# pkuyzy/ESC-GNN

Measured on AMD Instinct MI355X. Metric: graphs/sec + edges-aggregated/sec, NestedGIN_eff h=3 bs=128 @1/2/4/8 GPU, higher is better.
Workload: dtype f32; 1 GPU; count_cycle-shaped random regular graphs (n in 10/15/20/30), target=triangles, NestedGIN_eff h=3 layers=4 hidden=256, bs=128 per GPU (configs[1]); global_batch=128, parallelism=dp1 graph-sharded, rccl_ranks=1, ranks=1

## Files before the change

### esc-gnn_amd/csrc/linear_mfma.hip

```cpp
#include "common.h"
#include <cstdlib>
#include "linear_plan.h"
#include "gemm_tile.h"
#include "gemm_dma.h"
#include "linear_small.h"
#include "linear_narrow.h"

namespace esc {

using plan::Flags;
using plan::Op;
using plan::Plan;

static plan::PlanKnobs g_plan;
void set_linear_knob(int knob, int value) {
  if (knob == 11) g_plan.use_dma = value;
  else g_plan.knob[knob] = value;
}
static const plan::PlanKnobs& knobs() {
  static const bool env_read = [] {
    if (getenv("ESC_BIG_MIN_WGS")) g_plan.big_min_wgs = atoll(getenv("ESC_BIG_MIN_WGS"));
    if (getenv("ESC_TILE160")) g_plan.tile160 = atoi(getenv("ESC_TILE160"));
    if (getenv("ESC_TILE160_MIN_WGS")) g_plan.tile160_min_wgs = atoll(getenv("ESC_TILE160_MIN_WGS"));
    return true;
// ... 74 lines not shown
static void dma_fill_dw(dma::GArgs& g, const float* dY, int64_t ld_dy, const float* X, int64_t ld_x, const float* in_scale,
                        const float* in_shift, int64_t M, int64_t N, int64_t K, float* slabs, const Plan& p) {
  g.A = dY; g.lda = (int)ld_dy; g.B = X; g.ldb = (int)ld_x; g.C = slabs; g.ldc = (int)K;
  g.pro_scale = in_scale; g.pro_shift = in_shift; g.db_part = slabs + (size_t)p.splits * N * K;
  g.M = (int)N; g.N = (int)K; g.R = (int)M; g.red_per_split = p.per_split; g.accumulate = 0;
}

enum NarrowForm { NARROW_PLAIN, NARROW_FOLD, NARROW_L1 };
static void launch_narrow_fwd(NarrowForm form, const float* X, int64_t ld_x, const float* W, int64_t ld_w, const float* bias,
                              const float* in_scale, const float* in_shift, int64_t M, int64_t N, int64_t K, float* Y, int64_t ld_y,
                              const BnFoldDev& fold, const NarrowL1& l1, hipStream_t s) {
  const unsigned blocks = (unsigned)(cdiv(M, 16) < 2048 ? cdiv(M, 16) : 2048);
#define ESC_NARROW_FWD(...) \
  esc::launch(ESC_K_LINEAR, linear_narrow_fwd<__VA_ARGS__>, dim3(blocks), dim3(256), 0, s, X, ld_x, W, ld_w, bias, in_scale, in_shift, (int)M, (int)N, (int)K, Y, ld_y, fold, l1)
  if (form == NARROW_L1) ESC_NARROW_FWD(1, true, false, true);
  else if (form == NARROW_FOLD) { if (N == 1) ESC_NARROW_FWD(1, true, true); else ESC_NARROW_FWD(4, true, true); }
  else if (N == 1) { if (in_scale) ESC_NARROW_FWD(1, true); else ESC_NARROW_FWD(1, false); }
  else { if (in_scale) ESC_NARROW_FWD(4, true); else ESC_NARROW_FWD(4, false); }
#undef ESC_NARROW_FWD
}

static hipError_t launch_dma_fwd(const Plan& p, const dma::GArgs& g, hipStream_t s) {
  const bool pro = g.pro_scale != nullptr;
#define ESC_DMA_FWD(PRO, ...) dma::launch_gemm<__VA_ARGS__, false, false, PRO, true, false>(g, 0, s)
#define ESC_DMA_FWD_FROM(PRO, ...) dma::launch_gemm<__VA_ARGS__, false, false, PRO, true, false, true>(g, 0, s)
  const bool big = p.family == plan::F_DMA128;
  if (g.c_init != nullptr) {
    if (big) return pro ? ESC_DMA_FWD_FROM(1, ESC_T128) : ESC_DMA_FWD_FROM(0, ESC_T128);
    return pro ? ESC_DMA_FWD_FROM(1, ESC_T64) : ESC_DMA_FWD_FROM(0, ESC_T64);
  }
  if (g.fold.partials != nullptr) return big ? ESC_DMA_FWD(3, ESC_T128) : ESC_DMA_FWD(3, ESC_T64);
  switch (p.family) {
    case plan::F_DMA64X32:
      return pro ? dma::launch_gemm<ESC_T64X32, false, false, 1, false, false>(g, 0, s)
                 : dma::launch_gemm<ESC_T64X32, false, false, 0, false, false>(g, 0, s);
    case plan::F_DMA160: return pro ? ESC_DMA_FWD(1, ESC_T160) : ESC_DMA_FWD(0, ESC_T160);
    case plan::F_DMA128: return pro ? ESC_DMA_FWD(1, ESC_T128) : ESC_DMA_FWD(0, ESC_T128);
    case plan::F_DMA128X64: return ESC_DMA_FWD(0, ESC_T128X64);
    default: return pro ? ESC_DMA_FWD(1, ESC_T64) : ESC_DMA_FWD(0, ESC_T64);
  }
#undef ESC_DMA_FWD
#undef ESC_DMA_FWD_FROM
}
static dma::GArgs dma_fwd_args(const float* X, int64_t ld_x, const float* W, int64_t ld_w, const float* bias, const float* in_scale,
                               const float* in_shift, int64_t M, int64_t N, int64_t K, float* Y, int64_t ld_y, float* col_stats) {
  dma::GArgs g{};
  g.A = X; g.lda = (int)ld_x; g.B = W; g.ldb = (int)ld_w; g.C = Y; g.ldc = (int)ld_y; g.bias = bias;
  g.pro_scale = in_scale; g.pro_shift = in_shift; g.col_stats = reinterpret_cast<float2*>(col_stats);
  g.M = (int)M; g.N = (int)N; g.R = (int)K; g.red_per_split = (int)K; g.accumulate = 0;
  return g;
}

static int launch_smalln_dx(const float* dY, int64_t ld_dy, const float* W, int64_t ld_w, int64_t M, int64_t N, int64_t K, float* dX,
                            int64_t ld_dx, int accumulate, const BnbDev& bd, int act, const char* what, hipStream_t s) {
  const size_t lds = (size_t)(32 + small::SMALL_MAX) * (N + 4) * sizeof(float);
  static size_t raised[3] = {64 * 1024, 64 * 1024, 64 * 1024};
  hipError_t e = hipSuccess;
  if (act == 0) e = dma::raise_lds(small::smalln_dx<small::SMALL_MAX>, lds, raised[0]);
  if (act != 0) e = dma::raise_lds(small::smalln_dx<small::SMALL_MAX, 1>, lds, raised[1]);
  if (e == hipSuccess && act == 2) e = dma::raise_lds(small::smalln_dx<small::SMALL_MAX, 2>, lds, raised[2]);
  if (dma_check(e, what) != hipSuccess) return ESC_ELAUNCH;
  auto kern = act == 0 ? small::smalln_dx<small::SMALL_MAX> : (act == 2 ? small::smalln_dx<small::SMALL_MAX, 2> : small::smalln_dx<small::SMALL_MAX, 1>);
  esc::launch(ESC_K_LINEAR, kern, dim3((unsigned)cdiv(M, 32)), dim3(256), lds, s, dY, ld_dy, W, ld_w, (int)M, (int)N, (int)K, dX, ld_dx, accumulate, bd);
  return ESC_OK;
}

static void launch_wgrad_small(const float* dY, int64_t ld_dy, const float* X, int64_t ld_x, const float* in_scale, const float* in_shift,
                               int64_t M, int64_t N, int64_t K, float* slabs, const Plan& p, const BnbDev& bd, int act, hipStream_t s) {
  float* db_part = slabs + (size_t)p.splits * N * K;
  const bool small_k = K <= small::SMALL_MAX;
  const dim3 grid((unsigned)p.splits, (unsigned)cdiv(small_k ? N : K, 256));
#define ESC_WGRAD_SMALL(...) \
  esc::launch(ESC_K_LINEAR, small::wgrad_small<small::SMALL_MAX, __VA_ARGS__>, grid, dim3(256), 0, s, dY, ld_dy, X, ld_x, in_scale, in_shift, (int)M, (int)N, (int)K, slabs, db_part, bd)
  if (act == 2)      { if (in_scale) ESC_WGRAD_SMALL(true, true, 2); else ESC_WGRAD_SMALL(true, false, 2); }
  else if (act == 1) { if (in_scale) ESC_WGRAD_SMALL(true, true, 1); else ESC_WGRAD_SMALL(true, false, 1); }
  else if (small_k)  { if (in_scale) ESC_WGRAD_SMALL(true, true); else ESC_WGRAD_SMALL(true, false); }
  else               { if (in_scale) ESC_WGRAD_SMALL(false, true); else ESC_WGRAD_SMALL(false, false); }
#undef ESC_WGRAD_SMALL
}

static int reduce_slabs(const Plan& p, const float* slabs, int64_t N, int64_t K, float* dW, int64_t ld_dw, float* db, esc_reduce_job* defer,
                        void* stream) {
  esc_reduce_job now;
  esc_reduce_job* j = defer ? defer : &now;
  j->slabs = slabs; j->n = N * K; j->splits = p.splits; j->cols = K; j->dw = dW; j->ld_dw = ld_dw;
  j->db_part = slabs + (size_t)p.splits * N * K; j->rows = N; j->db = db;
  return defer ? ESC_OK : esc_slab_reduce_jobs(j, 1, stream);
}

}

using namespace esc;

extern "C" {

int esc_debug_gemm_occupancy(int tile_id) {
  int n = -1;
#define ESC_OCC(I)                                                                                                              \
  {                                                                                                                             \
    constexpr plan::Tile t = plan::R01_TILE[I];                                                                                 \
    auto kern = gemm_tile_kernel<t.bm, t.bn, t.wm, t.wn, t.bk, true, true, false, false>;                                       \
    const size_t lds = 2 * (KContigTile<t.bm, t.bk>::FLOATS + KContigTile<t.bn, t.bk>::FLOATS) * sizeof(float);                 \
    if (lds > 64 * 1024) (void)hipFuncSetAttribute((const void*)kern, hipFuncAttributeMaxDynamicSharedMemorySize, (int)lds);    \
    (void)hipOccupancyMaxActiveBlocksPerMultiprocessor(&n, kern, 256, lds);                                                     \
  }
  switch (tile_id) {
    case 0: ESC_OCC(0) break;
    case 2: ESC_OCC(2) break;
    case 3: ESC_OCC(3) break;
    case 4: ESC_OCC(4) break;
    default: ESC_OCC(1) break;
  }
#undef ESC_OCC
  return n;
}

static int linear_fwd_impl(const float* X, int64_t ld_x, const float* W, int64_t ld_w, const float* bias,
                           const float* in_scale, const float* in_shift, int64_t M, int64_t N, int64_t K,
                           float* Y, int64_t ld_y, float* col_stats, const esc_bn_fuse* bn, void* stream) {
  ESC_REQUIRE(X && W && Y, "esc_linear_fwd: null pointer");
  ESC_REQUIRE(M >= 0 && N > 0 && K > 0 && ld_x >= K && ld_w >= K && ld_y >= N, "esc_linear_fwd: bad sizes M=%ld N=%ld K=%ld", (long)M, (long)N, (long)K);
  ESC_REQUIRE((in_scale == nullptr) == (in_shift == nullptr), "esc_linear_fwd: in_scale/in_shift must come together");
  ESC_REQUIRE(col_stats == nullptr || N > 32, "esc_linear_fwd: col_stats needs N > 32");
  ESC_REQUIRE(M < (1LL << 31) && N < (1LL << 31) && K < (1LL << 31), "esc_linear_fwd: dimension too large");
  ESC_REQUIRE(bn == nullptr || (col_stats && bn->mean && bn->invstd && M > 1), "esc_linear_bn_fwd: needs col_stats, mean, invstd and M > 1");
  ESC_REQUIRE(bn == nullptr || ((bn->scale == nullptr) == (bn->shift == nullptr)), "esc_linear_bn_fwd: scale/shift must come together");
  if (M == 0) return ESC_OK;
  hipStream_t s = (hipStream_t)stream;
  Flags f = pro_flags(in_scale, in_shift);
  f.col_stats = col_stats != nullptr; f.bn = bn != nullptr; f.last_block_finalize = last_block_finalize();
  const Plan p = plan::plan_fwd(knobs(), Op{X, ld_x}, Op{W, ld_w}, M, N, K, f);
// ... 94 lines not shown
int esc_linear_fwd_from(const float* Y0, int64_t ld_y0, const float* X, int64_t ld_x, const float* W, int64_t ld_w, const float* bias,
                        const float* in_scale, const float* in_shift, int64_t M, int64_t N, int64_t K, float* Y, int64_t ld_y,
                        float* col_stats, void* stream) {
  ESC_REQUIRE(Y0 && X && W && Y, "esc_linear_fwd_from: null pointer");
  ESC_REQUIRE(M > 0 && N > 32 && K >= 32 && ld_y0 >= N && ld_x >= K && ld_w >= K && ld_y >= N && M < (1LL << 31), "esc_linear_fwd_from: bad sizes");
  ESC_REQUIRE((in_scale == nullptr) == (in_shift == nullptr), "esc_linear_fwd_from: in_scale/in_shift must come together");
  Flags f = pro_flags(in_scale, in_shift);
  f.c_init = true; f.col_stats = col_stats != nullptr;
  const Plan p = plan::plan_fwd(knobs(), Op{X, ld_x}, Op{W, ld_w}, M, N, K, f);
  ESC_REQUIRE(p.ok, "esc_linear_fwd_from: shape not served by the LDS-DMA tiles (M=%ld N=%ld K=%ld)", (long)M, (long)N, (long)K);
  dma::GArgs g = dma_fwd_args(X, ld_x, W, ld_w, bias, in_scale, in_shift, M, N, K, Y, ld_y, col_stats);
  g.c_init = Y0; g.ld_init = (int)ld_y0;
  return dma_check(launch_dma_fwd(p, g, (hipStream_t)stream), "esc_linear_fwd_from") == hipSuccess ? ESC_OK : ESC_ELAUNCH;
}
int esc_linear_fwd_from_ok(const float* X, int64_t ld_x, const float* W, int64_t ld_w, int64_t M, int64_t N, int64_t K, int has_prologue) {
  Flags f;
  f.pro = has_prologue != 0; f.c_init = true;
  return plan::plan_fwd(knobs(), Op{X, ld_x}, Op{W, ld_w}, M, N, K, f).ok ? 1 : 0;
}

int esc_linear_fwd_l1_ok(const float* X, int64_t ld_x, const float* w, int64_t K, const float* in_scale, const float* in_shift) {
  return (in_scale && in_shift && plan::plan_fwd(knobs(), Op{X, ld_x}, Op{w, K}, 1, 1, K, pro_flags(in_scale, in_shift)).family == plan::F_NARROW) ? 1 : 0;
}
int esc_linear_fwd_l1(const float* X, int64_t ld_x, const float* w, const float* bias, const float* in_scale, const float* in_shift,
                      int64_t M, int64_t K, const float* target, int64_t denom, float grad_scale, float* pred, float* dpred, void* stream) {
  ESC_REQUIRE(X && w && target && pred && dpred, "esc_linear_fwd_l1: null pointer");
  ESC_REQUIRE(M > 0 && K > 0 && ld_x >= K && denom > 0 && M < (1LL << 31), "esc_linear_fwd_l1: bad sizes");
  ESC_REQUIRE(in_scale != nullptr && in_shift != nullptr, "esc_linear_fwd_l1: the head reads pre-BatchNorm rows (in_scale / in_shift)");
  ESC_REQUIRE(esc_linear_fwd_l1_ok(X, ld_x, w, K, in_scale, in_shift), "esc_linear_fwd_l1: shape / alignment not served (K=%ld)", (long)K);
  const NarrowL1 l1{target, (float)((double)grad_scale / (double)denom), dpred};
  launch_narrow_fwd(NARROW_L1, X, ld_x, w, K, bias, in_scale, in_shift, M, 1, K, pred, 1, BnFoldDev{}, l1, (hipStream_t)stream);
  ESC_CHECK_LAUNCH("esc_linear_fwd_l1");
  return ESC_OK;
}

int esc_linear_bwd_input(const float* dY, int64_t ld_dy, const float* W, int64_t ld_w, int64_t M,
                         int64_t N, int64_t K, float* dX, int64_t ld_dx, int accumulate,
                         void* stream) {
  ESC_REQUIRE(dY && W && dX, "esc_linear_bwd_input: null pointer");
  ESC_REQUIRE(M >= 0 && N > 0 && K > 0 && ld_dy >= N && ld_w >= K && ld_dx >= K, "esc_linear_bwd_input: bad sizes");
  ESC_REQUIRE(M < (1LL << 31) && N < (1LL << 31) && K < (1LL << 31), "esc_linear_bwd_input: dimension too large");
  if (M == 0) return ESC_OK;
  hipStream_t s = (hipStream_t)stream;
  const Plan p = plan::plan_dx(knobs(), Op{dY, ld_dy}, Op{W, ld_w}, Op{dX, ld_dx}, M, N, K);
  switch (p.family) {
    case plan::F_NARROW_DX: {
      const unsigned blocks = (unsigned)(cdiv(M, 16) < 4096 ? cdiv(M, 16) : 4096);
      if (p.bn == 4) esc::launch(ESC_K_LINEAR, linear_narrow_dx<4>, dim3(blocks), dim3(256), 0, s, dY, ld_dy, W, ld_w, (int)M, (int)N, (int)K, dX, ld_dx, accumulate);
      else           esc::launch(ESC_K_LINEAR, linear_narrow_dx<16>, dim3(blocks), dim3(256), 0, s, dY, ld_dy, W, ld_w, (int)M, (int)N, (int)K, dX, ld_dx, accumulate);
      ESC_CHECK_LAUNCH("esc_linear_bwd_input.narrow");
      return ESC_OK;
    }
    case plan::F_SMALLN_DX:
      ESC_TRY_(launch_smalln_dx(dY, ld_dy, W, ld_w, M, N, K, dX, ld_dx, accumulate, BnbDev{}, 0, "esc_linear_bwd_input", s));
      ESC_CHECK_LAUNCH("esc_linear_bwd_input.smalln");
      return ESC_OK;
    case plan::F_DMA160_DX: case plan::F_DMA128_DX: case plan::F_DMA64_DX: {
      dma::GArgs d{};
      dma_fill_dx(d, dY, ld_dy, W, ld_w, M, N, K, dX, ld_dx, accumulate);
      const hipError_t e = p.family == plan::F_DMA160_DX   ? dma::launch_gemm<ESC_T160, false, true, 0, false, false>(d, 0, s)
                           : p.family == plan::F_DMA128_DX ? dma::launch_gemm<ESC_T128, false, true, 0, false, false>(d, 0, s)
                                                           : dma::launch_gemm<ESC_T64, false, true, 0, false, false>(d, 0, s);
      return dma_check(e, "esc_linear_bwd_input") == hipSuccess ? ESC_OK : ESC_ELAUNCH;
    }
    default:
      launch_r01<true, false, false, false>(p.tile, r01_dx_args(dY, ld_dy, W, ld_w, M, N, K, dX, ld_dx, accumulate), 1, s);
      ESC_CHECK_LAUNCH("esc_linear_bwd_input");
      return ESC_OK;
  }
}

int64_t esc_linear_bwd_weight_scratch(int64_t M, int64_t N, int64_t K) { return plan::bwd_weight_scratch(M, N, K); }

static int weight_impl(const float* dY, int64_t ld_dy, const float* X, int64_t ld_x, const float* in_scale,
                       const float* in_shift, int64_t M, int64_t N, int64_t K, float* dW, int64_t ld_dw, float* db,
                       float* slabs, esc_reduce_job* defer, void* stream) {
  ESC_REQUIRE(dY && X && dW && slabs, "esc_linear_bwd_weight: null pointer");
  ESC_REQUIRE(M > 0 && N > 0 && K > 0 && ld_dy >= N && ld_x >= K && ld_dw >= K, "esc_linear_bwd_weight: bad sizes");
  ESC_REQUIRE((in_scale == nullptr) == (in_shift == nullptr), "esc_linear_bwd_weight: in_scale/in_shift must come together");
  ESC_REQUIRE(M < (1LL << 31) && N < (1LL << 31) && K < (1LL << 31), "esc_linear_bwd_weight: dimension too large");
  hipStream_t s = (hipStream_t)stream;
  const Plan p = plan::plan_dw(knobs(), Op{dY, ld_dy}, Op{X, ld_x}, slabs, M, N, K);
  switch (p.family) {
    case plan::F_SMALL_DW:
      launch_wgrad_small(dY, ld_dy, X, ld_x, in_scale, in_shift, M, N, K, slabs, p, BnbDev{}, 0, s);
      ESC_CHECK_LAUNCH("esc_linear_bwd_weight.small");
      break;
    case plan::F_DMA128_DW: case plan::F_DMA64_DW: {
      dma::GArgs d{};
      dma_fill_dw(d, dY, ld_dy, X, ld_x, in_scale, in_shift, M, N, K, slabs, p);
      hipError_t e;
      if (p.family == plan::F_DMA128_DW) e = in_scale ? dma::launch_gemm<ESC_T128, true, true, 2, false, true>(d, 0, s)
                                                      : dma::launch_gemm<ESC_T128, true, true, 0, false, true>(d, 0, s);
      else                               e = in_scale ? dma::launch_gemm<ESC_T64, true, true, 2, false, true>(d, 0, s)
                                                      : dma::launch_gemm<ESC_T64, true, true, 0, false, true>(d, 0, s);
      if (dma_check(e, "esc_linear_bwd_weight") != hipSuccess) return ESC_ELAUNCH;
      break;
    }
    default: {
      const GemmArgs g = r01_dw_args(dY, ld_dy, X, ld_x, in_scale, in_shift, M, N, K, slabs, p);
      if (in_scale) launch_r01<false, false, true, true>(p.tile, g, p.splits, s);
      else          launch_r01<false, false, false, true>(p.tile, g, p.splits, s);
      ESC_CHECK_LAUNCH("esc_linear_bwd_weight.tiles");
    }
  }
  return reduce_slabs(p, slabs, N, K, dW, ld_dw, db, defer, stream);
}

int esc_linear_bwd_weight(const float* dY, int64_t ld_dy, const float* X, int64_t ld_x,
                          const float* in_scale, const float* in_shift, int64_t M, int64_t N,
                          int64_t K, float* dW, int64_t ld_dw, float* db, float* slabs,
                          void* stream) {
  return weight_impl(dY, ld_dy, X, ld_x, in_scale, in_shift, M, N, K, dW, ld_dw, db, slabs, nullptr, stream);
}

int esc_slab_reduce_jobs(const esc_reduce_job* jobs, int count, void* stream) {
  ESC_REQUIRE(jobs && count > 0 && count <= ESC_MAX_REDUCE_JOBS, "esc_slab_reduce_jobs: 1..%d jobs", ESC_MAX_REDUCE_JOBS);
  ReduceJobs t{};
  t.count = count;
  int blocks = 0;
  for (int j = 0; j < count; ++j) {
    ESC_REQUIRE(jobs[j].slabs && jobs[j].dw && jobs[j].n > 0 && jobs[j].splits > 0, "esc_slab_reduce_jobs: bad job %d", j);
    t.job[j] = jobs[j];
    t.block_start[j] = blocks;
    const esc_reduce_job& q = jobs[j];
    const bool vec = q.n % 4 == 0 && q.cols % 4 == 0 && q.ld_dw % 4 == 0 && aligned16(q.slabs) && aligned16(q.dw);
    t.vec[j] = vec ? 1 : 0;
    blocks += (int)(cdiv(vec ? q.n / 4 : q.n, 64) + (q.db ? cdiv(q.rows, 64) : 0));
  }
  t.block_start[count] = blocks;
  esc::launch(ESC_K_LINEAR, slab_reduce_multi_kernel, dim3((unsigned)blocks), dim3(256), 0, (hipStream_t)stream, t);
  ESC_CHECK_LAUNCH("esc_slab_reduce_jobs");
  return ESC_OK;
}

static int both_impl(const float* dY, int64_t ld_dy, const float* X, int64_t ld_x, const float* in_scale,
                     const float* in_shift, const float* W, int64_t ld_w, int64_t M, int64_t N, int64_t K,
                     float* dX, int64_t ld_dx, int accumulate, float* dW, int64_t ld_dw, float* db,
// ... 48 lines not shown
  }
  return reduce_slabs(p, slabs, N, K, dW, ld_dw, db, defer, stream);
}

int esc_linear_bwd_both(const float* dY, int64_t ld_dy, const float* X, int64_t ld_x, const float* in_scale,
                        const float* in_shift, const float* W, int64_t ld_w, int64_t M, int64_t N, int64_t K,
                        float* dX, int64_t ld_dx, int accumulate, float* dW, int64_t ld_dw, float* db,
                        float* slabs, void* stream) {
  return both_impl(dY, ld_dy, X, ld_x, in_scale, in_shift, W, ld_w, M, N, K, dX, ld_dx, accumulate, dW, ld_dw, db, slabs,
                   nullptr, stream);
}

int esc_linear_bwd_both_deferred(const float* dY, int64_t ld_dy, const float* X, int64_t ld_x, const float* in_scale,
                                 const float* in_shift, const float* W, int64_t ld_w, int64_t M, int64_t N, int64_t K,
                                 float* dX, int64_t ld_dx, int accumulate, float* dW, int64_t ld_dw, float* db,
                                 float* slabs, esc_reduce_job* job, void* stream) {
  ESC_REQUIRE(job, "esc_linear_bwd_both_deferred: null job");
  return both_impl(dY, ld_dy, X, ld_x, in_scale, in_shift, W, ld_w, M, N, K, dX, ld_dx, accumulate, dW, ld_dw, db, slabs,
                   job, stream);
}

static Plan plan_both_bn(const float* dOut, int64_t ld_dout, const esc_bn_bwd_fused* b, const float* X, int64_t ld_x, const float* W,
                         int64_t ld_w, int64_t M, int64_t N, int64_t K, const float* dX, int64_t ld_dx, const float* slabs,
                         const esc_bn_bwd_next* n) {
  plan::BnOps bo{};
  plan::NextOps no{};
  if (b) bo = plan::BnOps{b->x, b->ld_x, b->mean, b->invstd, b->scale, b->shift, b->coef, b->relu};
  if (n) no = plan::NextOps{n->partial, n->x, n->ld_x, n->mean, n->invstd, n->scale, n->shift, n->relu};
  return plan::plan_both_bn(knobs(), Op{dOut, ld_dout}, b ? &bo : nullptr, Op{X, ld_x}, Op{W, ld_w}, Op{dX, ld_dx}, slabs, n ? &no : nullptr,
                            M, N, K);
}

int esc_linear_bwd_both_bn_ok(const float* dOut, int64_t ld_dout, const esc_bn_bwd_fused* bn, const float* X, int64_t ld_x,
                              const float* W, int64_t ld_w, int64_t M, int64_t N, int64_t K, const float* dX, int64_t ld_dx,
                              const float* slabs, const esc_bn_bwd_next* next) {
  return plan_both_bn(dOut, ld_dout, bn, X, ld_x, W, ld_w, M, N, K, dX, ld_dx, slabs, next).ok ? 1 : 0;
}

int64_t esc_linear_bwd_bn_block_rows(int64_t M, int64_t N, int64_t K) { return plan::bwd_bn_block_rows(M, N, K); }

int esc_linear_bwd_both_bn(const float* dOut, int64_t ld_dout, const esc_bn_bwd_fused* bn, const float* X, int64_t ld_x,
                           const float* in_scale, const float* in_shift, const float* W, int64_t ld_w, int64_t M,
                           int64_t N, int64_t K, float* dX, int64_t ld_dx, int accumulate, float* dW, int64_t ld_dw,
                           float* db, float* slabs, esc_reduce_job* defer, const esc_bn_bwd_next* next, void* stream) {
  ESC_REQUIRE(dOut && X && W && dW && slabs, "esc_linear_bwd_both_bn: null pointer");
  ESC_REQUIRE((in_scale == nullptr) == (in_shift == nullptr), "esc_linear_bwd_both_bn: in_scale/in_shift must come together");
  ESC_REQUIRE(ld_dw >= K, "esc_linear_bwd_both_bn: bad sizes");
  const Plan p = plan_both_bn(dOut, ld_dout, bn, X, ld_x, W, ld_w, M, N, K, dX, ld_dx, slabs, next);
  ESC_REQUIRE(p.ok, "esc_linear_bwd_both_bn: shape / alignment not served (M=%ld N=%ld K=%ld) - use esc_bn_bwd + esc_linear_bwd_both", (long)M, (long)N, (long)K);
  hipStream_t s = (hipStream_t)stream;
  const BnbDev bd = bn ? BnbDev{bn->x, (int)bn->ld_x, bn->mean, bn->invstd, bn->scale, bn->shift, reinterpret_cast<const float2*>(bn->coef), bn->relu}
                       : BnbDev{};
  if (p.family == plan::F_SMALL_BN) {
    const int act = bd.relu == 2 ? 2 : 1;
    launch_wgrad_small(dOut, ld_dout, X, ld_x, in_scale, in_shift, M, N, K, slabs, p, bd, act, s);
    ESC_CHECK_LAUNCH("esc_linear_bwd_both_bn.small");
    if (dX != nullptr) {
      ESC_TRY_(launch_smalln_dx(dOut, ld_dout, W, ld_w, M, N, K, dX, ld_dx, accumulate, bd, act, "esc_linear_bwd_both_bn", s));
      ESC_CHECK_LAUNCH("esc_linear_bwd_both_bn.smalln");
    }
    return reduce_slabs(p, slabs, N, K, dW, ld_dw, db, defer, stream);
  }
  dma::DualArgs a{};
  dma_fill_dx(a.dx, dOut, ld_dout, W, ld_w, M, N, K, dX, ld_dx, accumulate);
  dma_fill_dw(a.dw, dOut, ld_dout, X, ld_x, in_scale, in_shift, M, N, K, slabs, p);
  a.dx.bnb = bd; a.dw.bnb = bd;
  if (next)
    a.dx.bst = BnStatDev{reinterpret_cast<float2*>(next->partial), next->x, (int)next->ld_x, next->mean, next->invstd, next->scale, next->shift, next->relu};
  hipError_t e;
#define ESC_T64_2STAGE 64, 64, 32, 2, 2, 2, 2
  if (p.family == plan::F_DMA128_BN) {
    if (next) e = in_scale ? dma::launch_dual<ESC_T128, true, true, true>(a, 0, s) : dma::launch_dual<ESC_T128, false, true, true>(a, 0, s);
    else      e = in_scale ? dma::launch_dual<ESC_T128, true, true, false>(a, 0, s) : dma::launch_dual<ESC_T128, false, true, false>(a, 0, s);
  } else {
    if (bn == nullptr) e = in_scale ? dma::launch_dual<ESC_T64, true, false, true>(a, 0, s) : dma::launch_dual<ESC_T64, false, false, true>(a, 0, s);
    else if (next)     e = in_scale ? dma::launch_dual<ESC_T64_2STAGE, true, true, true>(a, 0, s) : dma::launch_dual<ESC_T64_2STAGE, false, true, true>(a, 0, s);
    else               e = in_scale ? dma::launch_dual<ESC_T64_2STAGE, true, true, false>(a, 0, s) : dma::launch_dual<ESC_T64_2STAGE, false, true, false>(a, 0, s);
  }
#undef ESC_T64_2STAGE
  if (dma_check(e, "esc_linear_bwd_both_bn") != hipSuccess) return ESC_ELAUNCH;
  return reduce_slabs(p, slabs, N, K, dW, ld_dw, db, defer, stream);
}

}
```

### esc-gnn_amd/csrc/linear_small.h

```cpp
#pragma once
#include "common.h"
#include "linear_plan.h"

namespace esc {
namespace small {


template <int KMAX>
__global__ __launch_bounds__(256) void smallk_fwd(const float* __restrict__ X, int64_t ldx, const float* __restrict__ W,
                                                  int64_t ldw, const float* __restrict__ bias, int M, int N, int K,
                                                  float* __restrict__ Y, int64_t ldy, float2* __restrict__ col_stats) {
  ESC_PRIO();
  __shared__ float xs[ROWS_FWD * KMAX];
  const int n = blockIdx.y * 256 + threadIdx.x;
  const int r0 = blockIdx.x * ROWS_FWD;
  const int rows = min(ROWS_FWD, M - r0);
  for (int i = threadIdx.x; i < ROWS_FWD * KMAX; i += 256) {
    const int r = i / KMAX, k = i % KMAX;
    xs[i] = (r < rows && k < K) ? X[(size_t)(r0 + r) * ldx + k] : 0.f;
  }
  float w[KMAX];
#pragma unroll
  for (int k = 0; k < KMAX; ++k) w[k] = (n < N && k < K) ? W[(size_t)n * ldw + k] : 0.f;
  const float b = (bias != nullptr && n < N) ? bias[n] : 0.f;
  __syncthreads();
  if (n >= N) return;
  float y[ROWS_FWD];
  float s1 = 0.f;
#pragma unroll
  for (int r = 0; r < ROWS_FWD; ++r) {
    float a = b;
#pragma unroll
    for (int k = 0; k < KMAX; ++k) a = fmaf(xs[r * KMAX + k], w[k], a);
    y[r] = a;
    if (r < rows) { Y[(size_t)(r0 + r) * ldy + n] = a; s1 += a; }
  }
  if (col_stats != nullptr) {
    const float mean = s1 / (float)rows;
    float m2 = 0.f;
#pragma unroll
    for (int r = 0; r < ROWS_FWD; ++r)
      if (r < rows) { const float d = y[r] - mean; m2 = fmaf(d, d, m2); }
    col_stats[(size_t)blockIdx.x * N + n] = make_float2(mean, m2);
  }
}

template <int SMAX, bool SMALL_K, bool PRO, int BNB = 0>
__global__ __launch_bounds__(256) void wgrad_small(const float* __restrict__ dY, int64_t lddy, const float* __restrict__ X,
                                                   int64_t ldx, const float* __restrict__ sc, const float* __restrict__ sh,
                                                   int M, int N, int K, float* __restrict__ slabs, float* __restrict__ db_part,
                                                   BnbDev bnb) {
  static_assert(BNB == 0 || SMALL_K, "the fused BatchNorm backward transforms the wide dY operand");
  ESC_PRIO();
  __shared__ float us[ROWS_WGRAD * SMAX];
  const int t = blockIdx.y * 256 + threadIdx.x;
  const int split = blockIdx.x;
  const int r0 = split * ROWS_WGRAD;
  const int rows = min(ROWS_WGRAD, M - r0);
  const int S = SMALL_K ? K : N;
  const int Wd = SMALL_K ? N : K;
  const float* U = SMALL_K ? X : dY;
  const int64_t ldu = SMALL_K ? ldx : lddy;
  for (int i = threadIdx.x; i < rows * S; i += 256) {
    float v = U[(size_t)(r0 + i / S) * ldu + (i % S)];
    if constexpr (PRO && SMALL_K) v = fmaxf(fmaf(v, sc[i % S], sh[i % S]), 0.f);
    us[(i / S) * SMAX + (i % S)] = v;
  }
  for (int i = threadIdx.x; i < ROWS_WGRAD * SMAX; i += 256)
    if (i / SMAX >= rows || i % SMAX >= S) us[i] = 0.f;
  __syncthreads();
  float acc[SMAX];
#pragma unroll
  for (int q = 0; q < SMAX; ++q) acc[q] = 0.f;
  float colsum = 0.f;
  if (t < Wd) {
    const float* V = SMALL_K ? dY : X;
    const int64_t ldv = SMALL_K ? lddy : ldx;
    float psc = 1.f, psh = 0.f;
    if constexpr (PRO && !SMALL_K) { psc = sc[t]; psh = sh[t]; }
    float b_mu = 0.f, b_a = 0.f, b_ms = 0.f, b_mh = 1.f, b_k1 = 0.f, b_k2 = 0.f;
    if constexpr (BNB != 0) {
      const float2 kk = bnb.coef[t];
      b_mu = bnb.mean[t]; b_a = bnb.scale[t]; b_k1 = kk.x; b_k2 = bnb.invstd[t] * kk.y;
      if (bnb.relu) { b_ms = b_a; b_mh = bnb.shift[t]; }
    }
#pragma unroll 4
    for (int r = 0; r < rows; ++r) {
      float v = V[(size_t)(r0 + r) * ldv + t];
      if constexpr (BNB == 1) v = bnb_apply(v, bnb.x[(size_t)(r0 + r) * bnb.ldx + t], b_mu, b_a, b_ms, b_mh, b_k1, b_k2);
      if constexpr (BNB == 2) v = bnb_apply_elu(v, bnb.x[(size_t)(r0 + r) * bnb.ldx + t], b_mu, b_a, b_ms, b_mh, b_k1, b_k2);
      if constexpr (PRO && !SMALL_K) v = fmaxf(fmaf(v, psc, psh), 0.f);
      if constexpr (SMALL_K) colsum += v;
#pragma unroll
      for (int q = 0; q < SMAX; ++q) acc[q] = fmaf(us[r * SMAX + q], v, acc[q]);
    }
    float* out = slabs + (size_t)split * N * K;
#pragma unroll
    for (int q = 0; q < SMAX; ++q)
      if (q < S) out[SMALL_K ? (size_t)t * K + q : (size_t)q * K + t] = acc[q];
    if constexpr (SMALL_K) db_part[(size_t)split * N + t] = colsum;
  }
  if constexpr (!SMALL_K) {
    if (blockIdx.y == 0 && (int)threadIdx.x < N) {
      float s = 0.f;
      for (int r = 0; r < rows; ++r) s += us[r * SMAX + threadIdx.x];
      db_part[(size_t)split * N + threadIdx.x] = s;
    }
  }
}

template <int KMAX, int BNB = 0>
__global__ __launch_bounds__(256) void smalln_dx(const float* __restrict__ dY, int64_t lddy, const float* __restrict__ W,
                                                 int64_t ldw, int M, int N, int K, float* __restrict__ dX, int64_t lddx,
                                                 int accumulate, BnbDev bnb) {
  ESC_PRIO();
  extern __shared__ __attribute__((aligned(16))) float sm[];
  const int ldn = N + 4;
  float* ys = sm;
  float* wt = sm + 32 * ldn;
  const int r0 = blockIdx.x * 32;
  const int rows = min(32, M - r0);
  for (int i = threadIdx.x; i < rows * (N / 4); i += 256) {
    const int r = i / (N / 4), c = (i % (N / 4)) * 4;
    float4 v = *reinterpret_cast<const float4*>(dY + (size_t)(r0 + r) * lddy + c);
    if constexpr (BNB != 0) {
      const float4 x = *reinterpret_cast<const float4*>(bnb.x + (size_t)(r0 + r) * bnb.ldx + c);
      const float4 mu = *reinterpret_cast<const float4*>(bnb.mean + c), a = *reinterpret_cast<const float4*>(bnb.scale + c);
      const float4 is = *reinterpret_cast<const float4*>(bnb.invstd + c);
      const float4 k01 = *reinterpret_cast<const float4*>(bnb.coef + c), k23 = *reinterpret_cast<const float4*>(bnb.coef + c + 2);
      float4 ms = make_float4(0.f, 0.f, 0.f, 0.f), mh = make_float4(1.f, 1.f, 1.f, 1.f);
      if (bnb.relu) { ms = a; mh = *reinterpret_cast<const float4*>(bnb.shift + c); }
      if constexpr (BNB == 2) {
        v.x = bnb_apply_elu(v.x, x.x, mu.x, a.x, ms.x, mh.x, k01.x, is.x * k01.y); v.y = bnb_apply_elu(v.y, x.y, mu.y, a.y, ms.y, mh.y, k01.z, is.y * k01.w);
        v.z = bnb_apply_elu(v.z, x.z, mu.z, a.z, ms.z, mh.z, k23.x, is.z * k23.y); v.w = bnb_apply_elu(v.w, x.w, mu.w, a.w, ms.w, mh.w, k23.z, is.w * k23.w);
      } else {
        v.x = bnb_apply(v.x, x.x, mu.x, a.x, ms.x, mh.x, k01.x, is.x * k01.y); v.y = bnb_apply(v.y, x.y, mu.y, a.y, ms.y, mh.y, k01.z, is.y * k01.w);
        v.z = bnb_apply(v.z, x.z, mu.z, a.z, ms.z, mh.z, k23.x, is.z * k23.y); v.w = bnb_apply(v.w, x.w, mu.w, a.w, ms.w, mh.w, k23.z, is.w * k23.w);
      }
    }
    *reinterpret_cast<float4*>(ys + r * ldn + c) = v;
  }
  for (int i = threadIdx.x; i < N * K; i += 256) wt[(i % K) * ldn + (i / K)] = W[(size_t)(i / K) * ldw + (i % K)];
  __syncthreads();
  const int r = threadIdx.x >> 3, ks = threadIdx.x & 7;
  if (r >= rows) return;
#pragma unroll
  for (int kk = 0; kk < KMAX / 8; ++kk) {
    const int k = ks + kk * 8;
    if (k >= K) break;
    float a0 = 0.f, a1 = 0.f, a2 = 0.f, a3 = 0.f;
    for (int c = 0; c < N; c += 4) {
      const float4 y = *reinterpret_cast<const float4*>(ys + r * ldn + c);
      const float4 w = *reinterpret_cast<const float4*>(wt + k * ldn + c);
      a0 = fmaf(y.x, w.x, a0); a1 = fmaf(y.y, w.y, a1); a2 = fmaf(y.z, w.z, a2); a3 = fmaf(y.w, w.w, a3);
    }
    float v = (a0 + a1) + (a2 + a3);
    float* dst = dX + (size_t)(r0 + r) * lddx + k;
    if (accumulate) v += *dst;
    *dst = v;
  }
}

}
}
```

Before: 134,100 graphs/s.

## Fuse BatchNorm-backward weight and input gradients into one small-K kernel

Replaces the separate wgrad_small and smalln_dx launches on the BatchNorm-fused small path with a single bn_both kernel. It applies the BN backward transform to dOut once into LDS, computes the weight-gradient slab and bias partials, then reuses the transformed rows to compute dX against W staged in LDS. This avoids a second launch and re-reading dOut and the BN input x from global memory. Separately, the plain wgrad_small kernel now preloads its row values into registers ahead of the LDS staging. The cost is a larger LDS footprint per block and more register pressure.

```diff
diff --git a/esc-gnn_amd/csrc/linear_mfma.hip b/esc-gnn_amd/csrc/linear_mfma.hip
--- a/esc-gnn_amd/csrc/linear_mfma.hip
+++ b/esc-gnn_amd/csrc/linear_mfma.hip
@@ -150,31 +150,45 @@
 }
 
 static int launch_smalln_dx(const float* dY, int64_t ld_dy, const float* W, int64_t ld_w, int64_t M, int64_t N, int64_t K, float* dX,
-                            int64_t ld_dx, int accumulate, const BnbDev& bd, int act, const char* what, hipStream_t s) {
+                            int64_t ld_dx, int accumulate, const char* what, hipStream_t s) {
   const size_t lds = (size_t)(32 + small::SMALL_MAX) * (N + 4) * sizeof(float);
-  static size_t raised[3] = {64 * 1024, 64 * 1024, 64 * 1024};
-  hipError_t e = hipSuccess;
-  if (act == 0) e = dma::raise_lds(small::smalln_dx<small::SMALL_MAX>, lds, raised[0]);
-  if (act != 0) e = dma::raise_lds(small::smalln_dx<small::SMALL_MAX, 1>, lds, raised[1]);
-  if (e == hipSuccess && act == 2) e = dma::raise_lds(small::smalln_dx<small::SMALL_MAX, 2>, lds, raised[2]);
-  if (dma_check(e, what) != hipSuccess) return ESC_ELAUNCH;
-  auto kern = act == 0 ? small::smalln_dx<small::SMALL_MAX> : (act == 2 ? small::smalln_dx<small::SMALL_MAX, 2> : small::smalln_dx<small::SMALL_MAX, 1>);
-  esc::launch(ESC_K_LINEAR, kern, dim3((unsigned)cdiv(M, 32)), dim3(256), lds, s, dY, ld_dy, W, ld_w, (int)M, (int)N, (int)K, dX, ld_dx, accumulate, bd);
+  static size_t raised = 64 * 1024;
+  if (dma_check(dma::raise_lds(small::smalln_dx<small::SMALL_MAX>, lds, raised), what) != hipSuccess) return ESC_ELAUNCH;
+  esc::launch(ESC_K_LINEAR, small::smalln_dx<small::SMALL_MAX>, dim3((unsigned)cdiv(M, 32)), dim3(256), lds, s, dY, ld_dy, W, ld_w, (int)M, (int)N,
+              (int)K, dX, ld_dx, accumulate);
   return ESC_OK;
 }
 
 static void launch_wgrad_small(const float* dY, int64_t ld_dy, const float* X, int64_t ld_x, const float* in_scale, const float* in_shift,
-                               int64_t M, int64_t N, int64_t K, float* slabs, const Plan& p, const BnbDev& bd, int act, hipStream_t s) {
+                               int64_t M, int64_t N, int64_t K, float* slabs, const Plan& p, hipStream_t s) {
   float* db_part = slabs + (size_t)p.splits * N * K;
   const bool small_k = K <= small::SMALL_MAX;
   const dim3 grid((unsigned)p.splits, (unsigned)cdiv(small_k ? N : K, 256));
 #define ESC_WGRAD_SMALL(...) \
-  esc::launch(ESC_K_LINEAR, small::wgrad_small<small::SMALL_MAX, __VA_ARGS__>, grid, dim3(256), 0, s, dY, ld_dy, X, ld_x, in_scale, in_shift, (int)M, (int)N, (int)K, slabs, db_part, bd)
-  if (act == 2)      { if (in_scale) ESC_WGRAD_SMALL(true, true, 2); else ESC_WGRAD_SMALL(true, false, 2); }
-  else if (act == 1) { if (in_scale) ESC_WGRAD_SMALL(true, true, 1); else ESC_WGRAD_SMALL(true, false, 1); }
-  else if (small_k)  { if (in_scale) ESC_WGRAD_SMALL(true, true); else ESC_WGRAD_SMALL(true, false); }
-  else               { if (in_scale) ESC_WGRAD_SMALL(false, true); else ESC_WGRAD_SMALL(false, false); }
+  esc::launch(ESC_K_LINEAR, small::wgrad_small<small::SMALL_MAX, __VA_ARGS__>, grid, dim3(256), 0, s, dY, ld_dy, X, ld_x, in_scale, in_shift, (int)M, (int)N, (int)K, slabs, db_part)
+  if (small_k) { if (in_scale) ESC_WGRAD_SMALL(true, true); else ESC_WGRAD_SMALL(true, false); }
+  else         { if (in_scale) ESC_WGRAD_SMALL(false, true); else ESC_WGRAD_SMALL(false, false); }
 #undef ESC_WGRAD_SMALL
+}
+
+template <int BNB, bool PRO>
+static int launch_bn_both_as(const float* dOut, int64_t ld_dout, const float* X, int64_t ld_x, const float* in_scale, const float* in_shift,
+                             const float* W, int64_t ld_w, int64_t M, int64_t N, int64_t K, float* dX, int64_t ld_dx, int accumulate,
+                             float* slabs, const Plan& p, const BnbDev& bd, hipStream_t s) {
+  const size_t lds = (size_t)small::bn_both_lds_floats((int)N) * sizeof(float);
+  static size_t raised = 64 * 1024;
+  if (dma_check(dma::raise_lds(small::bn_both<small::SMALL_MAX, BNB, PRO>, lds, raised), "esc_linear_bwd_both_bn") != hipSuccess) return ESC_ELAUNCH;
+  esc::launch(ESC_K_LINEAR, small::bn_both<small::SMALL_MAX, BNB, PRO>, dim3((unsigned)p.splits), dim3(256), lds, s, dOut, ld_dout, X, ld_x, in_scale,
+              in_shift, W, ld_w, (int)M, (int)N, (int)K, dX, ld_dx, accumulate, slabs, slabs + (size_t)p.splits * N * K, bd);
+  return ESC_OK;
+}
+static int launch_bn_both(const float* dOut, int64_t ld_dout, const float* X, int64_t ld_x, const float* in_scale, const float* in_shift,
+                          const float* W, int64_t ld_w, int64_t M, int64_t N, int64_t K, float* dX, int64_t ld_dx, int accumulate, float* slabs,
+                          const Plan& p, const BnbDev& bd, hipStream_t s) {
+#define ESC_BN_BOTH(BNB, PRO) launch_bn_both_as<BNB, PRO>(dOut, ld_dout, X, ld_x, in_scale, in_shift, W, ld_w, M, N, K, dX, ld_dx, accumulate, slabs, p, bd, s)
+  if (bd.relu == 2) return in_scale ? ESC_BN_BOTH(2, true) : ESC_BN_BOTH(2, false);
+  return in_scale ? ESC_BN_BOTH(1, true) : ESC_BN_BOTH(1, false);
+#undef ESC_BN_BOTH
 }
 
 static int reduce_slabs(const Plan& p, const float* slabs, int64_t N, int64_t K, float* dW, int64_t ld_dw, float* db, esc_reduce_job* defer,
@@ -375,7 +389,7 @@
       return ESC_OK;
     }
     case plan::F_SMALLN_DX:
-      ESC_TRY_(launch_smalln_dx(dY, ld_dy, W, ld_w, M, N, K, dX, ld_dx, accumulate, BnbDev{}, 0, "esc_linear_bwd_input", s));
+      ESC_TRY_(launch_smalln_dx(dY, ld_dy, W, ld_w, M, N, K, dX, ld_dx, accumulate, "esc_linear_bwd_input", s));
       ESC_CHECK_LAUNCH("esc_linear_bwd_input.smalln");
       return ESC_OK;
     case plan::F_DMA160_DX: case plan::F_DMA128_DX: case plan::F_DMA64_DX: {
@@ -406,7 +420,7 @@
   const Plan p = plan::plan_dw(knobs(), Op{dY, ld_dy}, Op{X, ld_x}, slabs, M, N, K);
   switch (p.family) {
     case plan::F_SMALL_DW:
-      launch_wgrad_small(dY, ld_dy, X, ld_x, in_scale, in_shift, M, N, K, slabs, p, BnbDev{}, 0, s);
+      launch_wgrad_small(dY, ld_dy, X, ld_x, in_scale, in_shift, M, N, K, slabs, p, s);
       ESC_CHECK_LAUNCH("esc_linear_bwd_weight.small");
       break;
     case plan::F_DMA128_DW: case plan::F_DMA64_DW: {
@@ -561,13 +575,8 @@
   const BnbDev bd = bn ? BnbDev{bn->x, (int)bn->ld_x, bn->mean, bn->invstd, bn->scale, bn->shift, reinterpret_cast<const float2*>(bn->coef), bn->relu}
                        : BnbDev{};
   if (p.family == plan::F_SMALL_BN) {
-    const int act = bd.relu == 2 ? 2 : 1;
-    launch_wgrad_small(dOut, ld_dout, X, ld_x, in_scale, in_shift, M, N, K, slabs, p, bd, act, s);
+    ESC_TRY_(launch_bn_both(dOut, ld_dout, X, ld_x, in_scale, in_shift, W, ld_w, M, N, K, dX, ld_dx, accumulate, slabs, p, bd, s));
     ESC_CHECK_LAUNCH("esc_linear_bwd_both_bn.small");
-    if (dX != nullptr) {
-      ESC_TRY_(launch_smalln_dx(dOut, ld_dout, W, ld_w, M, N, K, dX, ld_dx, accumulate, bd, act, "esc_linear_bwd_both_bn", s));
-      ESC_CHECK_LAUNCH("esc_linear_bwd_both_bn.smalln");
-    }
     return reduce_slabs(p, slabs, N, K, dW, ld_dw, db, defer, stream);
   }
   dma::DualArgs a{};
diff --git a/esc-gnn_amd/csrc/linear_small.h b/esc-gnn_amd/csrc/linear_small.h
--- a/esc-gnn_amd/csrc/linear_small.h
+++ b/esc-gnn_amd/csrc/linear_small.h
@@ -45,12 +45,10 @@
   }
 }
 
-template <int SMAX, bool SMALL_K, bool PRO, int BNB = 0>
+template <int SMAX, bool SMALL_K, bool PRO>
 __global__ __launch_bounds__(256) void wgrad_small(const float* __restrict__ dY, int64_t lddy, const float* __restrict__ X,
                                                    int64_t ldx, const float* __restrict__ sc, const float* __restrict__ sh,
-                                                   int M, int N, int K, float* __restrict__ slabs, float* __restrict__ db_part,
-                                                   BnbDev bnb) {
-  static_assert(BNB == 0 || SMALL_K, "the fused BatchNorm backward transforms the wide dY operand");
+                                                   int M, int N, int K, float* __restrict__ slabs, float* __restrict__ db_part) {
   ESC_PRIO();
   __shared__ float us[ROWS_WGRAD * SMAX];
   const int t = blockIdx.y * 256 + threadIdx.x;
@@ -59,40 +57,37 @@
   const int rows = min(ROWS_WGRAD, M - r0);
   const int S = SMALL_K ? K : N;
   const int Wd = SMALL_K ? N : K;
+  const float* V = SMALL_K ? dY : X;
+  const int64_t ldv = SMALL_K ? lddy : ldx;
+  float v[ROWS_WGRAD];
+  float psc = 1.f, psh = 0.f;
+#pragma unroll
+  for (int r = 0; r < ROWS_WGRAD; ++r) v[r] = t < Wd ? V[(size_t)(r0 + min(r, rows - 1)) * ldv + t] : 0.f;
+  if constexpr (PRO && !SMALL_K) { if (t < Wd) { psc = sc[t]; psh = sh[t]; } }
   const float* U = SMALL_K ? X : dY;
   const int64_t ldu = SMALL_K ? ldx : lddy;
   for (int i = threadIdx.x; i < rows * S; i += 256) {
-    float v = U[(size_t)(r0 + i / S) * ldu + (i % S)];
-    if constexpr (PRO && SMALL_K) v = fmaxf(fmaf(v, sc[i % S], sh[i % S]), 0.f);
-    us[(i / S) * SMAX + (i % S)] = v;
+    float u = U[(size_t)(r0 + i / S) * ldu + (i % S)];
+    if constexpr (PRO && SMALL_K) u = fmaxf(fmaf(u, sc[i % S], sh[i % S]), 0.f);
+    us[(i / S) * SMAX + (i % S)] = u;
   }
   for (int i = threadIdx.x; i < ROWS_WGRAD * SMAX; i += 256)
     if (i / SMAX >= rows || i % SMAX >= S) us[i] = 0.f;
   __syncthreads();
-  float acc[SMAX];
-#pragma unroll
-  for (int q = 0; q < SMAX; ++q) acc[q] = 0.f;
-  float colsum = 0.f;
   if (t < Wd) {
-    const float* V = SMALL_K ? dY : X;
-    const int64_t ldv = SMALL_K ? lddy : ldx;
-    float psc = 1.f, psh = 0.f;
-    if constexpr (PRO && !SMALL_K) { psc = sc[t]; psh = sh[t]; }
-    float b_mu = 0.f, b_a = 0.f, b_ms = 0.f, b_mh = 1.f, b_k1 = 0.f, b_k2 = 0.f;
-    if constexpr (BNB != 0) {
-      const float2 kk = bnb.coef[t];
-      b_mu = bnb.mean[t]; b_a = bnb.scale[t]; b_k1 = kk.x; b_k2 = bnb.invstd[t] * kk.y;
-      if (bnb.relu) { b_ms = b_a; b_mh = bnb.shift[t]; }
-    }
-#pragma unroll 4
-    for (int r = 0; r < rows; ++r) {
-      float v = V[(size_t)(r0 + r) * ldv + t];
-      if constexpr (BNB == 1) v = bnb_apply(v, bnb.x[(size_t)(r0 + r) * bnb.ldx + t], b_mu, b_a, b_ms, b_mh, b_k1, b_k2);
-      if constexpr (BNB == 2) v = bnb_apply_elu(v, bnb.x[(size_t)(r0 + r) * bnb.ldx + t], b_mu, b_a, b_ms, b_mh, b_k1, b_k2);
-      if constexpr (PRO && !SMALL_K) v = fmaxf(fmaf(v, psc, psh), 0.f);
-      if constexpr (SMALL_K) colsum += v;
-#pragma unroll
-      for (int q = 0; q < SMAX; ++q) acc[q] = fmaf(us[r * SMAX + q], v, acc[q]);
+    float acc[SMAX];
+#pragma unroll
+    for (int q = 0; q < SMAX; ++q) acc[q] = 0.f;
+    float colsum = 0.f;
+#pragma unroll
+    for (int r = 0; r < ROWS_WGRAD; ++r) {
+      if (r < rows) {
+        float x = v[r];
+        if constexpr (PRO && !SMALL_K) x = fmaxf(fmaf(x, psc, psh), 0.f);
+        if constexpr (SMALL_K) colsum += x;
+#pragma unroll
+        for (int q = 0; q < SMAX; ++q) acc[q] = fmaf(us[r * SMAX + q], x, acc[q]);
+      }
     }
     float* out = slabs + (size_t)split * N * K;
 #pragma unroll
@@ -109,10 +104,10 @@
   }
 }
 
-template <int KMAX, int BNB = 0>
+template <int KMAX>
 __global__ __launch_bounds__(256) void smalln_dx(const float* __restrict__ dY, int64_t lddy, const float* __restrict__ W,
                                                  int64_t ldw, int M, int N, int K, float* __restrict__ dX, int64_t lddx,
-                                                 int accumulate, BnbDev bnb) {
+                                                 int accumulate) {
   ESC_PRIO();
   extern __shared__ __attribute__((aligned(16))) float sm[];
   const int ldn = N + 4;
@@ -122,23 +117,7 @@
   const int rows = min(32, M - r0);
   for (int i = threadIdx.x; i < rows * (N / 4); i += 256) {
     const int r = i / (N / 4), c = (i % (N / 4)) * 4;
-    float4 v = *reinterpret_cast<const float4*>(dY + (size_t)(r0 + r) * lddy + c);
-    if constexpr (BNB != 0) {
-      const float4 x = *reinterpret_cast<const float4*>(bnb.x + (size_t)(r0 + r) * bnb.ldx + c);
-      const float4 mu = *reinterpret_cast<const float4*>(bnb.mean + c), a = *reinterpret_cast<const float4*>(bnb.scale + c);
-      const float4 is = *reinterpret_cast<const float4*>(bnb.invstd + c);
-      const float4 k01 = *reinterpret_cast<const float4*>(bnb.coef + c), k23 = *reinterpret_cast<const float4*>(bnb.coef + c + 2);
-      float4 ms = make_float4(0.f, 0.f, 0.f, 0.f), mh = make_float4(1.f, 1.f, 1.f, 1.f);
-      if (bnb.relu) { ms = a; mh = *reinterpret_cast<const float4*>(bnb.shift + c); }
-      if constexpr (BNB == 2) {
-        v.x = bnb_apply_elu(v.x, x.x, mu.x, a.x, ms.x, mh.x, k01.x, is.x * k01.y); v.y = bnb_apply_elu(v.y, x.y, mu.y, a.y, ms.y, mh.y, k01.z, is.y * k01.w);
-        v.z = bnb_apply_elu(v.z, x.z, mu.z, a.z, ms.z, mh.z, k23.x, is.z * k23.y); v.w = bnb_apply_elu(v.w, x.w, mu.w, a.w, ms.w, mh.w, k23.z, is.w * k23.w);
-      } else {
-        v.x = bnb_apply(v.x, x.x, mu.x, a.x, ms.x, mh.x, k01.x, is.x * k01.y); v.y = bnb_apply(v.y, x.y, mu.y, a.y, ms.y, mh.y, k01.z, is.y * k01.w);
-        v.z = bnb_apply(v.z, x.z, mu.z, a.z, ms.z, mh.z, k23.x, is.z * k23.y); v.w = bnb_apply(v.w, x.w, mu.w, a.w, ms.w, mh.w, k23.z, is.w * k23.w);
-      }
-    }
-    *reinterpret_cast<float4*>(ys + r * ldn + c) = v;
+    *reinterpret_cast<float4*>(ys + r * ldn + c) = *reinterpret_cast<const float4*>(dY + (size_t)(r0 + r) * lddy + c);
   }
   for (int i = threadIdx.x; i < N * K; i += 256) wt[(i % K) * ldn + (i / K)] = W[(size_t)(i / K) * ldw + (i % K)];
   __syncthreads();
@@ -161,5 +140,174 @@
   }
 }
 
-}
-}
+__host__ __device__ constexpr int bn_both_lds_floats(int N) {
+  return (32 + SMALL_MAX) * (N + 4) > 32 * (N + 4) + ROWS_WGRAD * SMALL_MAX ? (32 + SMALL_MAX) * (N + 4) : 32 * (N + 4) + ROWS_WGRAD * SMALL_MAX;
+}
+
+template <int SMAX, int BNB, bool PRO>
+__global__ __launch_bounds__(256) void bn_both(const float* __restrict__ dOut, int64_t lddo, const float* __restrict__ X, int64_t ldx,
+                                               const float* __restrict__ sc, const float* __restrict__ sh, const float* __restrict__ W,
+                                               int64_t ldw, int M, int N, int K, float* __restrict__ dX, int64_t lddx, int accumulate,
+                                               float* __restrict__ slabs, float* __restrict__ db_part, BnbDev bnb) {
+  static_assert(BNB == 1 || BNB == 2, "the plain gradients are wgrad_small and smalln_dx");
+  static_assert(ROWS_WGRAD == 32, "a slab is the 32-row block of the dX rows");
+  ESC_PRIO();
+  extern __shared__ __attribute__((aligned(16))) float sm[];
+  const int ldn = N + 4;
+  float* ys = sm;
+  float* wt = sm + 32 * ldn;
+  const int xs_off = bn_both_lds_floats(N) - ROWS_WGRAD * SMAX;
+  float* xs = sm + xs_off;
+  const bool w_early = dX != nullptr && (32 + K) * ldn <= xs_off;
+  const int tid = threadIdx.x;
+  const int split = blockIdx.x;
+  const int r0 = split * ROWS_WGRAD;
+  const int rows = min(ROWS_WGRAD, M - r0);
+  const int nk = N * K;
+  auto load_w = [&](int i0, float (&w)[16]) {
+#pragma unroll
+    for (int u = 0; u < 16; ++u) { const int i = i0 + 256 * u; w[u] = i < nk ? W[(size_t)(i / K) * ldw + (i % K)] : 0.f; }
+  };
+  auto store_w = [&](int i0, const float (&w)[16]) {
+#pragma unroll
+    for (int u = 0; u < 16; ++u) { const int i = i0 + 256 * u; if (i < nk) wt[(i % K) * ldn + (i / K)] = w[u]; }
+  };
+  auto stage_w = [&](int from) {
+    for (int i0 = from; i0 < nk; i0 += 256 * 16) { float w[16]; load_w(i0, w); store_w(i0, w); }
+  };
+
+  const int G = N >> 2;
+  const int rpp = 256 / G;
+  const int rin = tid / G, c = (tid - rin * G) * 4;
+  const bool stager = rin < rpp;
+  const int passes = (rows + rpp - 1) / rpp;
+  float4 g[8], x[8];
+  auto load_batch = [&](int p0) {
+#pragma unroll
+    for (int u = 0; u < 8; ++u) {
+      const int r = (p0 + u) * rpp + rin;
+      g[u] = x[u] = make_float4(0.f, 0.f, 0.f, 0.f);
+      if (stager && r < rows) {
+        g[u] = *reinterpret_cast<const float4*>(dOut + (size_t)(r0 + r) * lddo + c);
+        x[u] = *reinterpret_cast<const float4*>(bnb.x + (size_t)(r0 + r) * bnb.ldx + c);
+      }
+    }
+  };
+  load_batch(0);
+  float a_next = tid < N ? bnb.scale[tid] : 0.f;
+  const int cl = stager ? c : 0;
+  const float4 mu = *reinterpret_cast<const float4*>(bnb.mean + cl), is = *reinterpret_cast<const float4*>(bnb.invstd + cl);
+  const float4 k01 = *reinterpret_cast<const float4*>(bnb.coef + cl), k23 = *reinterpret_cast<const float4*>(bnb.coef + cl + 2);
+  float4 ms = make_float4(0.f, 0.f, 0.f, 0.f), mh = make_float4(1.f, 1.f, 1.f, 1.f);
+  if (bnb.relu) { ms = *reinterpret_cast<const float4*>(bnb.scale + cl); mh = *reinterpret_cast<const float4*>(bnb.shift + cl); }
+  float xv[ROWS_WGRAD * SMAX / 256];
+#pragma unroll
+  for (int u = 0; u < ROWS_WGRAD * SMAX / 256; ++u) {
+    const int i = tid + 256 * u, r = i / SMAX, q = i % SMAX;
+    xv[u] = 0.f;
+    if (r < rows && q < K) {
+      xv[u] = X[(size_t)(r0 + r) * ldx + q];
+      if constexpr (PRO) xv[u] = fmaxf(fmaf(xv[u], sc[q], sh[q]), 0.f);
+    }
+  }
+  if (w_early) {
+    float w[16];
+    load_w(tid, w);
+    store_w(tid, w);
+    stage_w(tid + 256 * 16);
+  }
+#pragma unroll
+  for (int u = 0; u < ROWS_WGRAD * SMAX / 256; ++u) xs[tid + 256 * u] = xv[u];
+  const float4 k1 = make_float4(k01.x, k01.z, k23.x, k23.z);
+  const float4 k2 = make_float4(is.x * k01.y, is.y * k01.w, is.z * k23.y, is.w * k23.w);
+  for (int p0 = 0;;) {
+#pragma unroll
+    for (int u = 0; u < 8; ++u) {
+      const int r = (p0 + u) * rpp + rin;
+      if (stager && r < rows) {
+        float4 f;
+        if constexpr (BNB == 2) {
+          f.x = bnb_apply_elu(g[u].x, x[u].x, mu.x, 1.f, ms.x, mh.x, k1.x, k2.x); f.y = bnb_apply_elu(g[u].y, x[u].y, mu.y, 1.f, ms.y, mh.y, k1.y, k2.y);
+          f.z = bnb_apply_elu(g[u].z, x[u].z, mu.z, 1.f, ms.z, mh.z, k1.z, k2.z); f.w = bnb_apply_elu(g[u].w, x[u].w, mu.w, 1.f, ms.w, mh.w, k1.w, k2.w);
+        } else {
+          f.x = bnb_apply(g[u].x, x[u].x, mu.x, 1.f, ms.x, mh.x, k1.x, k2.x); f.y = bnb_apply(g[u].y, x[u].y, mu.y, 1.f, ms.y, mh.y, k1.y, k2.y);
+          f.z = bnb_apply(g[u].z, x[u].z, mu.z, 1.f, ms.z, mh.z, k1.z, k2.z); f.w = bnb_apply(g[u].w, x[u].w, mu.w, 1.f, ms.w, mh.w, k1.w, k2.w);
+        }
+        *reinterpret_cast<float4*>(ys + r * ldn + c) = f;
+      }
+    }
+    p0 += 8;
+    if (p0 >= passes) break;
+    load_batch(p0);
+  }
+  __syncthreads();
+
+  for (int t = tid; t < N; t += 256) {
+    const float a = a_next;
+    if (t + 256 < N) a_next = bnb.scale[t + 256];
+    int xo = xs_off;
+    asm volatile("" : "+v"(xo));
+    const float* xs = sm + xo;
+    float acc[SMAX];
+#pragma unroll
+    for (int q = 0; q < SMAX; ++q) acc[q] = 0.f;
+    float colsum = 0.f;
+    if (rows == ROWS_WGRAD) {
+      float f[ROWS_WGRAD];
+#pragma unroll
+      for (int r = 0; r < ROWS_WGRAD; ++r) f[r] = ys[r * ldn + t];
+      if (dX != nullptr) {
+#pragma unroll
+        for (int r = 0; r < ROWS_WGRAD; ++r) ys[r * ldn + t] = a * f[r];
+      }
+#pragma unroll
+      for (int r = 0; r < ROWS_WGRAD; ++r) {
+        const float v = a * f[r];
+        colsum = fmaf(a, f[r], colsum);
+#pragma unroll
+        for (int q = 0; q < SMAX; ++q) acc[q] = fmaf(xs[r * SMAX + q], v, acc[q]);
+      }
+    } else {
+      for (int r = 0; r < rows; ++r) {
+        const float f = ys[r * ldn + t];
+        const float v = a * f;
+        colsum = fmaf(a, f, colsum);
+#pragma unroll
+        for (int q = 0; q < SMAX; ++q) acc[q] = fmaf(xs[r * SMAX + q], v, acc[q]);
+        if (dX != nullptr) ys[r * ldn + t] = v;
+      }
+    }
+    float* out = slabs + (size_t)split * N * K;
+#pragma unroll
+    for (int q = 0; q < SMAX; ++q)
+      if (q < K) out[(size_t)t * K + q] = acc[q];
+    db_part[(size_t)split * N + t] = colsum;
+  }
+  if (dX == nullptr) return;
+  __syncthreads();
+  if (!w_early) {
+    stage_w(tid);
+    __syncthreads();
+  }
+
+  const int r = tid >> 3, ks = tid & 7;
+  if (r >= rows) return;
+#pragma unroll
+  for (int kk = 0; kk < SMAX / 8; ++kk) {
+    const int k = ks + kk * 8;
+    if (k >= K) break;
+    float a0 = 0.f, a1 = 0.f, a2 = 0.f, a3 = 0.f;
+    for (int cc = 0; cc < N; cc += 4) {
+      const float4 y = *reinterpret_cast<const float4*>(ys + r * ldn + cc);
+      const float4 w = *reinterpret_cast<const float4*>(wt + k * ldn + cc);
+      a0 = fmaf(y.x, w.x, a0); a1 = fmaf(y.y, w.y, a1); a2 = fmaf(y.z, w.z, a2); a3 = fmaf(y.w, w.w, a3);
+    }
+    float v = (a0 + a1) + (a2 + a3);
+    float* dst = dX + (size_t)(r0 + r) * lddx + k;
+    if (accumulate) v += *dst;
+    *dst = v;
+  }
+}
+
+}
+}
```

New measurement: 134,900 graphs/s (median of 6 runs). About the same (+0.6%).
